# amorim-cleison/sign-language-nlp

Measured on AMD Instinct MI355X. Metric: train seq/s (batch=50,len=48), higher is better.
Workload: dtype bf16x3; 1 GPU; cfg2: Transformer train step E512 H8 N6 F512 batch 50 len 48 |src| 3000 |tgt| 202 dropout 0.1, fwd+CE+bwd+clip(0.5)+SGD(m=.9); launch=eager stream launches (auto: timed both in 9 untimed pre-warmup steps + warmup), per_gpu=independent fit (grid shard)

## Files before the change

### include/slnlp.h

```cpp
#ifndef SLNLP_H
#define SLNLP_H

#include <stdint.h>

#ifdef __cplusplus
extern "C" {
#endif

#define SLNLP_OK 0
#define SLNLP_ERR_INVALID_ARG 1
#define SLNLP_ERR_LAUNCH 2
#define SLNLP_ERR_UNSUPPORTED 3

#define SLNLP_ABI_VERSION 1

const char* slnlp_last_error(void);
int slnlp_abi_version(void);

typedef struct slnlp_gemm_args {
    const float* A; int64_t lda; int32_t a_kmajor;
    const float* B; int64_t ldb; int32_t b_kmajor;
    float* C; int64_t ldc;
    int32_t M, N, K;
    const float* bias;
// ... 5 lines not shown
    int32_t precision;
    int32_t gate_mode;
    const uint16_t* A_hi; const uint16_t* A_lo; int64_t lda_p;
    const uint16_t* B_hi; const uint16_t* B_lo; int64_t ldb_p;
    uint16_t* C_hi; uint16_t* C_lo; int64_t ldc_p;
    int32_t drop_head_dim;
    const float* col_scale;
    uint8_t* C_q8;
    int32_t batch;
    int64_t batch_stride_a, batch_stride_b, batch_stride_c;
} slnlp_gemm_args;

int slnlp_gemm(const slnlp_gemm_args* args, void* stream);
int64_t slnlp_gemm_group_scratch_bytes(const slnlp_gemm_args* jobs, const int32_t* split_k, int njobs);
int slnlp_set_plane_tile(int tile);
int slnlp_set_gemm_ks(int ks);
int slnlp_set_rnn_step_tile(int rows16);
int slnlp_set_fp8_tile(int tile);
int slnlp_gemm_group(const slnlp_gemm_args* jobs, const int32_t* split_k, int njobs, void* scratch,
                     int64_t scratch_bytes, void* stream);
int slnlp_gemm_wd(const slnlp_gemm_args* wgrad, const slnlp_gemm_args* dgrad, void* scratch, int64_t scratch_bytes, void* stream);
int slnlp_gemm_wd_plan(const slnlp_gemm_args* wgrad, const slnlp_gemm_args* dgrad, int32_t* split, int32_t* separate, int32_t* geo_wgrad,
                       int32_t* geo_dgrad);
int slnlp_gemm_rows(const slnlp_gemm_args* args, void* stream);
int slnlp_gemm_rows_ln(const slnlp_gemm_args* args, const float* x, int64_t ldx, const float* gamma, const float* beta, float eps,
                       float* y, float* stats, uint16_t* y_hi, uint16_t* y_lo, int64_t ldp, void* stream);
int slnlp_gemm_rows_bwd(const slnlp_gemm_args* dgrad, const slnlp_gemm_args* wgrad, void* stream);
int slnlp_set_rows_tile(int tile);
int slnlp_quant_rows_fp8(const float* x, int64_t ld, int R, int K, uint8_t* q, int64_t ldq, float* scale, void* stream);
int slnlp_split_planes(const float* x, int64_t ld, int R, int C, uint16_t* hi, uint16_t* lo, int64_t ldp, void* stream);
// ... 518 lines not shown
```

### sign-language-nlp_amd/csrc/gemm_planes.hip

```cpp
#include <algorithm>
#include <vector>

#include "common.hpp"
#include "gemm_jobs.hpp"

namespace slnlp {

typedef __attribute__((ext_vector_type(8))) __bf16 bf16x8;
typedef __attribute__((ext_vector_type(4))) short s16x4;
typedef __attribute__((ext_vector_type(8))) short s16x8;
typedef __attribute__((ext_vector_type(4))) float f32x4;
typedef __attribute__((address_space(3))) void* lds_vp;
typedef __attribute__((address_space(1))) const void* glb_vp;
typedef __attribute__((ext_vector_type(4))) unsigned int u32x4;

constexpr int PT = 64;
constexpr int PTHREADS = 512;

__device__ __forceinline__ int mswz(int k) { return (((k >> 1) & 1) | (((k >> 3) & 1) << 1)) << 1; }

template <bool KMAJOR>
__device__ __forceinline__ int img_off(int row, int k) {
    if (KMAJOR) return row * PT + ((((k >> 3) ^ (row & 7)) << 3) | (k & 7));
    return k * PT + ((((row >> 3) ^ mswz(k)) << 3) | (row & 7));
// ... 71 lines not shown
#define TS_CLK(slot) do { } while (0)
#else
#define TS_CLK(slot) do { if (slot == 1) ts[6] = __builtin_amdgcn_s_memtime(); if (slot == 2) ts[7] = __builtin_amdgcn_s_memtime(); } while (0)
#endif
#define TS_MARK(slot) do { if (threadIdx.x == 0) { ts[slot] = __builtin_amdgcn_s_memrealtime(); \
        TS_CLK(slot); } } while (0)
#else
#define TS_MARK(slot) do { } while (0)
#endif
#if SLNLP_PROBE_FENCES == 128 && defined(SLNLP_PROBE_EPI)
#define TS_EPI(slot) do { if (threadIdx.x == 0) ts[slot] = __builtin_amdgcn_s_memrealtime(); } while (0)
#else
#define TS_EPI(slot) do { } while (0)
#endif

template <int NSPLIT, bool AK, bool BK, int BM, int BN, int BKS, int NST>
__device__ __forceinline__ void plane_kloop(const slnlp_gemm_args& g, unsigned short* smem, int bm0, int bn0, int kt0, int kt1,
                                            bool do_rowsum, f32x4 (&acc)[BM / 64][BN / 32], float (&rowsum)[BM / PT],
                                            unsigned long long* ts) {
    constexpr int NPA = NSPLIT == 3 ? 2 : 1, NPB = NSPLIT >= 2 ? 2 : 1;
    constexpr int SUBM = BM / PT, SUBN = BN / PT;
    constexpr int MT = BM / 64, NT = BN / 32;
    constexpr int IMG_E = PT * BKS;
    constexpr int A_IMGS = NPA * SUBM, B_IMGS = NPB * SUBN;
    constexpr int STAGE = (A_IMGS + B_IMGS) * IMG_E;
    constexpr int PIECES = (A_IMGS + B_IMGS) * BKS / 64;
    static_assert(BKS == 64 || (BM % 128 == 0 && BN % 128 == 0), "32-k stages move 128-row slabs");
    const int tid = threadIdx.x, lane = tid & 63, wave = __builtin_amdgcn_readfirstlane(tid >> 6);
    const int wm0 = (wave >> 1) * (BM / 4), wn0 = (wave & 1) * (BN / 2);
    const int am_last = ((g.M + PT - 1) / PT - 1) * PT, bn_last = ((g.N + PT - 1) / PT - 1) * PT;

    constexpr int APC = BKS == 64 ? SUBM : SUBM / 2, BPC = BKS == 64 ? SUBN : SUBN / 2;
    unsigned aoff[APC], boff[BPC];
#pragma unroll
    for (int q = 0; q < APC; ++q) {
        if constexpr (BKS == 64) aoff[q] = plane_lane_off<AK>(g.lda_p, BM > PT ? min(bm0 + q * PT, am_last) : bm0, wave, lane);
        else aoff[q] = slab32_lane_off<AK>(g.lda_p, bm0 + 2 * q * PT, am_last, wave, lane);
    }
#pragma unroll
    for (int q = 0; q < BPC; ++q) {
        if constexpr (BKS == 64) boff[q] = plane_lane_off<BK>(g.ldb_p, BN > PT ? min(bn0 + q * PT, bn_last) : bn0, wave, lane);
        else boff[q] = slab32_lane_off<BK>(g.ldb_p, bn0 + 2 * q * PT, bn_last, wave, lane);
    }
    constexpr int PSTEP = BKS == 64 ? 1 : 2;
    auto issue = [&](int kt, int stage) {
        const int k0 = (kt < kt1 ? kt : kt0) * BKS;
        const long ka = AK ? (long)k0 : (long)k0 * g.lda_p, kb = BK ? (long)k0 : (long)k0 * g.ldb_p;
        unsigned short* s = smem + stage * STAGE + wave * 512;
#pragma unroll
        for (int q = 0; q < APC; ++q) {
            dma_piece(g.A_hi, ka, aoff[q], s + q * PSTEP * IMG_E);
            if (NPA == 2) dma_piece(g.A_lo, ka, aoff[q], s + (SUBM + q * PSTEP) * IMG_E);
        }
#pragma unroll
        for (int q = 0; q < BPC; ++q) {
            dma_piece(g.B_hi, kb, boff[q], s + (A_IMGS + q * PSTEP) * IMG_E);
            if (NPB == 2) dma_piece(g.B_lo, kb, boff[q], s + (A_IMGS + SUBN + q * PSTEP) * IMG_E);
        }
    };

    for (int t = 0; t < NST - 1; ++t) issue(kt0 + t, t);
    for (int kt = kt0; kt < kt1; ++kt) {
        const int it = kt - kt0;
        asm volatile("s_waitcnt vmcnt(%0)\n\ts_waitcnt lgkmcnt(0)" ::"n"((NST - 2) * PIECES) : "memory");
        __builtin_amdgcn_s_barrier();
        asm volatile("" ::: "memory");
#if SLNLP_PROBE_FENCES == 128
        if (kt == kt0) TS_MARK(1);
#endif
        issue(kt + NST - 1, (it + NST - 1) % NST);
        const unsigned short* s = smem + (it % NST) * STAGE;
#pragma unroll
        for (int kk = 0; kk < BKS / 32; ++kk) {
            constexpr int JB = NT > 4 ? 4 : NT;
            bf16x8 ah[MT], al[MT];
#pragma unroll
            for (int i = 0; i < MT; ++i) {
                const int row = wm0 + 16 * i;
                if constexpr (BKS == 64) {
                    ah[i] = pfrag<AK>(s + (row / PT) * IMG_E, row % PT, kk, lane);
                    if (NPA == 2) al[i] = pfrag<AK>(s + (SUBM + row / PT) * IMG_E, row % PT, kk, lane);
                } else {
                    ah[i] = pfrag32<AK>(s + (row / PT) * IMG_E, row % PT, lane);
                    if (NPA == 2) al[i] = pfrag32<AK>(s + (SUBM + row / PT) * IMG_E, row % PT, lane);
                }
            }
#pragma unroll
            for (int j0 = 0; j0 < NT; j0 += JB) {
                bf16x8 bh[JB], bl[JB];
#pragma unroll
                for (int j = 0; j < JB; ++j) {
                    const int row = wn0 + 16 * (j0 + j);
                    if constexpr (BKS == 64) {
                        bh[j] = pfrag<BK>(s + (A_IMGS + row / PT) * IMG_E, row % PT, kk, lane);
                        if (NPB == 2) bl[j] = pfrag<BK>(s + (A_IMGS + SUBN + row / PT) * IMG_E, row % PT, kk, lane);
                    } else {
                        bh[j] = pfrag32<BK>(s + (A_IMGS + row / PT) * IMG_E, row % PT, lane);
                        if (NPB == 2) bl[j] = pfrag32<BK>(s + (A_IMGS + SUBN + row / PT) * IMG_E, row % PT, lane);
                    }
                }
#pragma unroll
                for (int i = 0; i < MT; ++i)
#pragma unroll
                    for (int j = 0; j < JB; ++j) {
                        f32x4& c = acc[i][j0 + j];
                        if (NPA == 2) c = __builtin_amdgcn_mfma_f32_16x16x32_bf16(al[i], bh[j], c, 0, 0, 0);
                        if (NPB == 2) c = __builtin_amdgcn_mfma_f32_16x16x32_bf16(ah[i], bl[j], c, 0, 0, 0);
                        c = __builtin_amdgcn_mfma_f32_16x16x32_bf16(ah[i], bh[j], c, 0, 0, 0);
                    }
            }
        }
        if (do_rowsum) {
            constexpr int OCT = BKS / 8;
            const int row = tid & 63, kq = ((tid >> 6) % OCT) * 8, sub0 = (tid >> 6) / OCT;
#pragma unroll
            for (int sm = 0; sm < SUBM; sm += 8 / OCT) {
                const int im = sm + sub0;
                float t = 0.f;
#pragma unroll
                for (int k = 0; k < 8; ++k) {
                    const int off = BKS == 64 ? img_off<AK>(row, kq + k) : img32_off<AK>(row, kq + k);
                    t += pbf2f(s[im * IMG_E + off]);
                    if (NPA == 2) t += pbf2f(s[(SUBM + im) * IMG_E + off]);
                }
                if (BKS == 64) rowsum[sm] += t;
                else if (kt & 1) rowsum[sm + 1] += t;
                else rowsum[sm] += t;
            }
        }
    }
}

template <int NSPLIT, int BM, int BN, int BKS, int NST>
__device__ __forceinline__ void plane_tile(const PlaneJob& job, int lid, bool placed, unsigned short* smem) {
    unsigned long long* tsp = nullptr;
#if SLNLP_PROBE_FENCES == 128
    unsigned long long ts[TS_W] = {0, 0, 0, 0, 0, 0, 0, 0};
    struct TsFlush {
        unsigned long long* t;
        __device__ ~TsFlush() {
            if (threadIdx.x == 0) {
                t[4] = __builtin_amdgcn_s_memrealtime();
                unsigned hw;
                asm volatile("s_getreg_b32 %0, hwreg(HW_REG_XCC_ID)" : "=s"(hw));
                t[5] = ((unsigned long long)hw << 32) | blockIdx.x;
                const unsigned i = atomicAdd(&g_ts_n, 1u) & (unsigned)(TS_MAX - 1);
                for (int k = 0; k < TS_W; ++k) g_ts[i][k] = t[k];
            }
        }
    } ts_flush{ts};
    tsp = ts;
    TS_MARK(0);
#endif
    constexpr int SUBM = BM / PT;
    constexpr int MT = BM / 64, NT = BN / 32;
    constexpr int KSUB = PT / BKS;
    const slnlp_gemm_args& g = job.a;
    const int tid = threadIdx.x, lane = tid & 63, wave = __builtin_amdgcn_readfirstlane(tid >> 6);
    const int wm0 = (wave >> 1) * (BM / 4), wn0 = (wave & 1) * (BN / 2);
    const int nks = job.nks;
    int bx, by, ks, tile;
    {
        const int nwg = job.tiles_x * job.tiles_y * nks;
        const int xcd = lid & 7, q = nwg >> 3, r = nwg & 7;
        const int t = placed ? lid : (xcd < r ? xcd * (q + 1) : r * (q + 1) + (xcd - r) * q) + (lid >> 3);
        const int ntiles = job.tiles_x * job.tiles_y;
        ks = t / ntiles;
        tile = t - ks * ntiles;
        constexpr int GR = BM >= 256 ? 2 : BM >= 128 ? 4 : 8;
        const int grp = tile / (GR * job.tiles_x), rem = tile - grp * (GR * job.tiles_x);
        const int rows_here = min(GR, job.tiles_y - grp * GR);
        bx = rem / rows_here;
        by = grp * GR + (rem - bx * rows_here);
        tile = by * job.tiles_x + bx;
// ... 1 lines not shown
    const int bm0 = by * BM, bn0 = bx * BN;
    const int M = g.M, N = g.N, K = g.K;
    const int ktiles = (K + PT - 1) / PT;
    const int kt0 = (int)((long)ktiles * ks / nks) * KSUB, kt1 = (int)((long)ktiles * (ks + 1) / nks) * KSUB;

    f32x4 acc[MT][NT];
#pragma unroll
    for (int i = 0; i < MT; ++i)
#pragma unroll
        for (int j = 0; j < NT; ++j) acc[i][j] = f32x4{0.f, 0.f, 0.f, 0.f};
    const bool do_rowsum = (g.rowsum_a != nullptr) && (bx == 0);
    float rowsum[SUBM];
#pragma unroll
    for (int i = 0; i < SUBM; ++i) rowsum[i] = 0.f;

    if (job.variant == 0) plane_kloop<NSPLIT, true, true, BM, BN, BKS, NST>(g, smem, bm0, bn0, kt0, kt1, do_rowsum, acc, rowsum, tsp);
    else if (job.variant == 1) plane_kloop<NSPLIT, true, false, BM, BN, BKS, NST>(g, smem, bm0, bn0, kt0, kt1, do_rowsum, acc, rowsum, tsp);
    else if (job.variant == 2) plane_kloop<NSPLIT, false, false, BM, BN, BKS, NST>(g, smem, bm0, bn0, kt0, kt1, do_rowsum, acc, rowsum, tsp);
    else if constexpr (NSPLIT == 3) {
        if (job.variant == 3) plane_kloop<2, true, false, BM, BN, BKS, NST + 1>(g, smem, bm0, bn0, kt0, kt1, do_rowsum, acc, rowsum, tsp);
        else plane_kloop<2, false, false, BM, BN, BKS, NST + 1>(g, smem, bm0, bn0, kt0, kt1, do_rowsum, acc, rowsum, tsp);
    }
    TS_MARK(2);
    asm volatile("s_waitcnt vmcnt(0)" ::: "memory");
    __builtin_amdgcn_s_barrier();
    float* rs = reinterpret_cast<float*>(smem);
    int* flag = reinterpret_cast<int*>(smem) + SUBM * PTHREADS;
    float rs_row = 0.f;
    if (do_rowsum) {
        if (BKS == 64) {
#pragma unroll
            for (int sm = 0; sm < SUBM; ++sm) rs[(sm * 8 + (tid >> 6)) * PT + (tid & 63)] = rowsum[sm];
        } else {
#pragma unroll
            for (int sm = 0; sm < SUBM; sm += 2) {
                const int im = sm + (tid >> 8), o = (tid >> 6) & 3;
// ... 74 lines not shown
    if (g.drop_p > 0.f) dkey = dropout_key(g.rng, g.drop_site);
#pragma unroll 1
    for (int ch = 0; ch < ECH; ++ch) {
        __syncthreads();
        if (ECH == 1 || wm0 / ER == ch) {
            const int lr0 = wm0 - ch * ER + crow, lc0 = wn0 + ccol;
#pragma unroll
            for (int i = 0; i < MT; ++i)
#pragma unroll
                for (int j = 0; j < NT; ++j)
#pragma unroll
                    for (int r = 0; r < 4; ++r) stg[(lr0 + 16 * i + r) * SLD + lc0 + 16 * j] = acc[i][j][r];
#if defined(SLNLP_PROBE_EPI) && SLNLP_PROBE_EPI == 2
            if (ch == 0) TS_EPI(6);
#endif
            if (early) {
                static_assert(NT % 2 == 0, "column tiles in pairs");
#pragma unroll 1
                for (int t = 0; t < MT * (NT / 2); ++t) {
                    const int lm0 = lr0 + 16 * (t / (NT / 2)), ln0 = lc0 + 32 * (t % (NT / 2));
                    const int gm0 = bm0 + ch * ER + lm0, gn0 = bn0 + ln0;
                    if (gn0 >= N || gm0 >= M) continue;
                    float v[2][4], gt[2][4];
#pragma unroll
                    for (int h = 0; h < 2; ++h)
#pragma unroll
                        for (int r = 0; r < 4; ++r) {
                            v[h][r] = stg[(lm0 + r) * SLD + ln0 + 16 * h];
                            gt[h][r] = 1.f;
                            if (g.gate && gm0 + r < M && gn0 + 16 * h < N) gt[h][r] = g.gate[(long)(gm0 + r) * g.ldg + gn0 + 16 * h];
                        }
// ... 269 lines not shown
                if (g.C) g.C[(long)gm * g.ldc + gn] = v;
                if (g.C_hi) {
                    unsigned short h, l;
                    split_bf16(v, h, l);
                    g.C_hi[(long)gm * g.ldc_p + gn] = h;
                    if (g.C_lo) g.C_lo[(long)gm * g.ldc_p + gn] = l;
                }
                if (g.C_q8) g.C_q8[(long)gm * g.ldc_p + gn] = (unsigned char)(pack_fp8x4(v, 0.f, 0.f, 0.f) & 0xFFu);
            }
        }
}

constexpr int PLACE_JOB_BITS = 12, PLACE_JOBS = 1 << PLACE_JOB_BITS;

struct GeoInfo { int bm, bn, bks, nst; };
constexpr int NGEO = 4;
constexpr GeoInfo GEO[NGEO] = {{64, 64, 64, 2}, {128, 128, 64, 2}, {128, 128, 32, 2}, {256, 256, 32, 2}};

template <int NSPLIT, int G>
__global__ __launch_bounds__(PTHREADS) void gemm_planes_kernel(const PlaneGroupParams P, const PlaneJob* __restrict__ tab,
                                                               const int* __restrict__ blockmap) {
    extern __shared__ __attribute__((aligned(16))) unsigned short smem[];
    PlaneJob job;
    int lid;
    bool placed = false;
    if (tab) {
        const int m = blockmap[blockIdx.x];
        if (m < 0) return;
        job = tab[m & (PLACE_JOBS - 1)];
        lid = m >> PLACE_JOB_BITS;
        placed = true;
    } else {
// ... 15 lines not shown
constexpr size_t plane_lds(int geo) {
    const size_t ring3 = (size_t)GEO[geo].nst * 2 * (GEO[geo].bm + GEO[geo].bn) * GEO[geo].bks * sizeof(unsigned short);
    const size_t ring2 = (size_t)(GEO[geo].nst + 1) * (GEO[geo].bm + 2 * GEO[geo].bn) * GEO[geo].bks * sizeof(unsigned short);
    const size_t ring = ring3 > ring2 ? ring3 : ring2;
    const size_t image = ((size_t)(GEO[geo].bm > 128 ? 128 : GEO[geo].bm) * (GEO[geo].bn + 4) + GEO[geo].bn) * sizeof(float);
    return ring > image ? ring : image;
}
constexpr int GROUP_COUNTERS = 4096;

struct Q8GeoInfo { int bm, bn, nst; };
constexpr int NQGEO = 2;
constexpr Q8GeoInfo QGEO[NQGEO] = {{64, 64, 4}, {128, 128, 2}};

template <int G>
__global__ __launch_bounds__(PTHREADS) void plane_splitk_reduce_kernel(const PlaneJob job_in) {
    constexpr int BM = GEO[G].bm, BN = GEO[G].bn, MT = BM / 64, NT = BN / 32, TILE_FLOATS = BM * BN, SC = 17;
    PlaneJob job = job_in;
    launder(job.a);
    const slnlp_gemm_args& g = job.a;
    const int tid = threadIdx.x, lane = tid & 63, wave = tid >> 6;
    const int tile = blockIdx.x / (MT * NT), slab = blockIdx.x - tile * (MT * NT), i = slab / NT, j = slab - i * NT;
    const int by = tile / job.tiles_x, bx = tile - by * job.tiles_x, nks = job.nks;
    const int wm0 = (wave >> 1) * (BM / 4), wn0 = (wave & 1) * (BN / 2);
    u32x4 p[WD_MAX_SPLITK];
#pragma unroll
    for (int s = 0; s < WD_MAX_SPLITK; ++s) {
        if (s < nks) {
            const __amdgpu_buffer_rsrc_t q =
                __builtin_amdgcn_make_buffer_rsrc(job.part + ((long)tile * nks + s) * TILE_FLOATS, 0, TILE_FLOATS * 4, 0x00020000);
            p[s] = __builtin_amdgcn_raw_buffer_load_b128(q, tid * 16, slab * PTHREADS * 16, SC);
// ... 56 lines not shown
static int q8_geo_of_knob(int knob) { return knob == 64 ? 0 : knob == 128 ? 1 : -1; }
static std::atomic<int> g_q8_geo{[] { const char* e = getenv("SLNLP_Q8_TILE"); return q8_geo_of_knob(e ? atoi(e) : 0); }()};
static int q8_geo_auto(const PlaneJob* jobs, int njobs) {
    const int forced = g_q8_geo.load(std::memory_order_relaxed);
    if (forced >= 0) return forced;
    long units = 0;
    for (int i = 0; i < njobs; ++i) units += (long)ceil_div(jobs[i].a.M, 128) * ceil_div(jobs[i].a.N, 128);
    return units >= 512 ? 1 : 0;
}

static int splitk_mode() {
    static const int mode = [] { const char* e = getenv("SLNLP_SPLITK_MODE"); return e ? atoi(e) : 0; }();
    return mode;
}

static int geo_of_knob(int knob) { return knob == 64 ? 0 : knob == 128 ? 1 : knob == 12832 ? 2 : knob == 256 ? 3 : -1; }
static std::atomic<int> g_plane_geo{[] { const char* e = getenv("SLNLP_PLANE_TILE"); return geo_of_knob(e ? atoi(e) : 0); }()};
constexpr int BIG_TILE_MIN_UNITS = 200;

constexpr int TWO_PER_CU_UNITS = 300;
struct LaunchShape {
    long units128 = 0, units256 = 0;
    int min_k = 1 << 30;
    bool forward = true;
    int njobs = 0;
};
static void shape_add(LaunchShape& s, const slnlp_gemm_args& a, int nks) {
    if (nks < 1) nks = 1;
    s.units128 += (long)ceil_div(a.M, 128) * ceil_div(a.N, 128) * nks;
    s.units256 += (long)ceil_div(a.M, 256) * ceil_div(a.N, 256) * nks;
    s.min_k = std::min(s.min_k, a.K / nks);
    s.forward = s.forward && a.a_kmajor && a.b_kmajor && nks == 1 && a.precision != 2;
    ++s.njobs;
}
static int plane_geo_auto(const LaunchShape& s) {
    const int forced = g_plane_geo.load(std::memory_order_relaxed);
    if (forced >= 0) return forced;
    if (s.units128 < BIG_TILE_MIN_UNITS) return 0;
    if (s.forward && s.min_k >= 1024 && (s.units256 >= 512 || s.min_k >= 2048) && s.units256 * 100 >= (s.units256 + 255) / 256 * 256 * 85) return 3;
    if (s.njobs == 1 && !s.forward && s.min_k >= 2048 && s.units256 >= 192 && s.units256 * 100 >= (s.units256 + 255) / 256 * 256 * 85) return 3;
    return (s.min_k >= 1024 || s.units128 >= TWO_PER_CU_UNITS) ? 2 : 1;
}
int plane_geo_for(const slnlp_gemm_args* jobs, const int* split_k, int njobs) {
    LaunchShape s;
    for (int i = 0; i < njobs; ++i) {
        if (jobs[i].precision == 8) return 0;
        shape_add(s, jobs[i], split_k ? split_k[i] : 1);
    }
    return plane_geo_auto(s);
}

int gemm_planes_init() {
    static DeviceOnce once;
    return once.run([]() -> int {
        bool ok = true;
        for (int prec = 1; prec <= 3; prec += 2)
            for (int geo = 0; geo < NGEO; ++geo)
                ok = ok && hipFuncSetAttribute(gemm_planes_kernel_ptr(prec, geo), hipFuncAttributeMaxDynamicSharedMemorySize, (int)plane_lds(geo)) == hipSuccess;
        for (int geo = 0; geo < NQGEO; ++geo)
            ok = ok && hipFuncSetAttribute(q8_kernel_ptr(geo), hipFuncAttributeMaxDynamicSharedMemorySize, (int)q8_lds(geo)) == hipSuccess;
        if (!ok) {
            set_error("gemm_planes_init: cannot raise dynamic LDS limit: %s", hipGetErrorString(hipGetLastError()));
            return SLNLP_ERR_LAUNCH;
        }
        return 0;
    });
}

static int check_plane_job(const slnlp_gemm_args& a) {
    SLNLP_CHECK_ARG(a.A_hi && a.B_hi, "gemm_planes: operand planes required");
    SLNLP_CHECK_ARG(a.C || a.C_hi, "gemm_planes: no output");
    SLNLP_CHECK_ARG(a.M > 0 && a.N > 0 && a.K > 0, "gemm_planes: bad shape M=%d N=%d K=%d", a.M, a.N, a.K);
    if (a.precision == 8) {
        SLNLP_CHECK_ARG(a.a_kmajor && a.b_kmajor, "gemm_planes: precision 8 (fp8) is built for k-major operands (forward products)");
        SLNLP_CHECK_ARG(a.lda_p % 128 == 0 && a.ldb_p % 128 == 0 && a.lda_p >= a.K && a.ldb_p >= a.K,
                        "gemm_planes: fp8 plane row strides must be multiples of 128 bytes and cover K");
        SLNLP_CHECK_ARG(!a.gate && !a.rowsum_a && a.drop_head_dim == 0, "gemm_planes: fp8 jobs take bias / relu / dropout / residual only");
        SLNLP_CHECK_ARG((((uintptr_t)a.A_hi | (uintptr_t)a.B_hi) & 15) == 0, "gemm_planes: planes must be 16-byte aligned");
// ... 318 lines not shown
    if (hipLaunchKernel(b.fn, dim3(blocks), dim3(PTHREADS), args, b.lds, s) != hipSuccess) {
        set_error("gemm_planes (batch): %s", hipGetErrorString(hipGetLastError()));
        return SLNLP_ERR_LAUNCH;
    }
    if (timed >= 0) launch_timer_end(timed, s, blocks, (int)b.jobs.size(), b.geo);
    return 0;
}
int plane_geo_forced() { return g_plane_geo.load(std::memory_order_relaxed); }

template <int NSPLIT>
static const void* kernel_of(int geo) {
    switch (geo) {
        case 1: return (const void*)gemm_planes_kernel<NSPLIT, 1>;
        case 2: return (const void*)gemm_planes_kernel<NSPLIT, 2>;
        case 3: return (const void*)gemm_planes_kernel<NSPLIT, 3>;
        default: return (const void*)gemm_planes_kernel<NSPLIT, 0>;
    }
}
const void* gemm_planes_kernel_ptr(int precision, int geo) { return precision == 1 ? kernel_of<1>(geo) : kernel_of<3>(geo); }

int gemm_planes(const slnlp_gemm_args& a, hipStream_t s) { return gemm_planes_group(&a, nullptr, 1, nullptr, 0, s); }

__device__ __forceinline__ void split_planes_body(const float* __restrict__ x, long ld, int R, int C, unsigned short* __restrict__ hi,
                                                  unsigned short* __restrict__ lo, long ldp) {
    const long n4 = (long)R * (C >> 2);
    for (long i = blockIdx.x * 256L + threadIdx.x; i < n4; i += (long)gridDim.x * 256) {
        const int r = (int)(i / (C >> 2)), c = (int)(i % (C >> 2)) << 2;
        const float4 v = *reinterpret_cast<const float4*>(x + (long)r * ld + c);
        const float f[4] = {v.x, v.y, v.z, v.w};
        unsigned short h[4], l[4];
// ... 45 lines not shown
                   hipStream_t st) {
    SLNLP_CHECK_ARG(x && q && scale && R > 0, "quant_rows_fp8: bad arguments");
    SLNLP_CHECK_ARG(row_table || (K > 0 && K % 4 == 0 && ld % 4 == 0 && ldq % 4 == 0 && ldq >= K), "quant_rows_fp8: K, ld, ldq must be multiples of 4");
    return zlaunch(quant_rows_fp8_kernel, dim3(ceil_div(R, 4)), 256, 0, st, "quant_rows_fp8", x, (long)ld, R, K, q, (long)ldq, scale,
                   (const QuantRow*)row_table);
}

}

extern "C" int slnlp_quant_rows_fp8(const float* x, int64_t ld, int R, int K, uint8_t* q, int64_t ldq, float* scale, void* stream) {
    return slnlp::quant_rows_fp8(x, ld, R, K, q, ldq, scale, nullptr, (hipStream_t)stream);
}

extern "C" int slnlp_set_plane_tile(int tile) {
    if (tile != 0 && slnlp::geo_of_knob(tile) < 0) {
        slnlp::set_error("set_plane_tile: %d (0 = automatic, 64, 128, 12832 = 128 x 128 with 32-k stages, 256 = 256 x 256 with 32-k stages)", tile);
        return SLNLP_ERR_INVALID_ARG;
    }
    slnlp::g_plane_geo.store(slnlp::geo_of_knob(tile), std::memory_order_relaxed);
    return 0;
}

extern "C" int slnlp_set_fp8_tile(int tile) {
    if (tile != 0 && slnlp::q8_geo_of_knob(tile) < 0) {
        slnlp::set_error("set_fp8_tile: %d (0 = automatic, 64 or 128)", tile);
        return SLNLP_ERR_INVALID_ARG;
    }
    slnlp::g_q8_geo.store(slnlp::q8_geo_of_knob(tile), std::memory_order_relaxed);
    return 0;
}

extern "C" int64_t slnlp_gemm_group_scratch_bytes(const slnlp_gemm_args* jobs, const int32_t* split_k, int njobs) {
    if (!jobs || njobs < 1) return 0;
    return (int64_t)slnlp::gemm_group_scratch_bytes(jobs, split_k, njobs);
}
// ... 50 lines not shown
```

### sign-language-nlp_amd/slnlp/_lib.py

```python
import ctypes as C
import os

_HERE = os.path.dirname(os.path.abspath(__file__))
LIB_PATH = os.path.join(os.path.dirname(_HERE), "lib",
                        f"libslnlp_probe{os.environ['SLNLP_PROBE_LIB']}.so" if os.environ.get("SLNLP_PROBE_LIB") else "libslnlp.so")

i32, i64, f32, vp = C.c_int32, C.c_int64, C.c_float, C.c_void_p


class GemmArgs(C.Structure):
    _fields_ = [("A", vp), ("lda", i64), ("a_kmajor", i32),
                ("B", vp), ("ldb", i64), ("b_kmajor", i32),
                ("C", vp), ("ldc", i64),
                ("M", i32), ("N", i32), ("K", i32),
                ("bias", vp), ("relu", i32),
                ("gate", vp), ("ldg", i64), ("gate_scale", f32),
                ("drop_p", f32), ("drop_site", i32), ("rng", vp),
                ("resid", vp), ("ldr", i64),
                ("rowsum_a", vp), ("precision", i32), ("gate_mode", i32),
                ("A_hi", vp), ("A_lo", vp), ("lda_p", i64), ("B_hi", vp), ("B_lo", vp), ("ldb_p", i64),
                ("C_hi", vp), ("C_lo", vp), ("ldc_p", i64), ("drop_head_dim", i32),
                ("col_scale", vp), ("C_q8", vp),
                ("batch", i32), ("batch_stride_a", i64), ("batch_stride_b", i64), ("batch_stride_c", i64)]

# ... 196 lines not shown
    "slnlp_tf_debug_layout": (i32, [vp, C.c_char_p, i64]),
    "slnlp_tf_set_destroy_sync": (i32, [vp, i32]),
    "slnlp_tf_set_criterion": (i32, [vp, vp, f32, i32, vp]),
    "slnlp_tf_set_update": (i32, [vp, i32, f32, f32, i32]),
    "slnlp_tf_set_param_groups": (i32, [vp, i32, vp, vp, i32, vp, vp, vp]),
    "slnlp_tf_set_averaging": (i32, [vp, vp, vp, i32, f32]),
    "slnlp_tf_set_dmem_batched": (i32, [vp, i32]),
    "slnlp_tf_set_dec_ln_fused": (i32, [vp, i32]),
    "slnlp_set_stream_policy": (i32, [i32]),
    "slnlp_set_thread_stream_policy": (i32, [i32]),
    "slnlp_set_backward_passes": (i32, [i32, i32]),
    "slnlp_get_backward_passes": (i32, [C.POINTER(i32), C.POINTER(i32)]),
    "slnlp_launch_timer_start": (i32, [i32]),
    "slnlp_launch_timer_stop": (i32, [C.POINTER(TimedLaunch), i32]),
    "slnlp_set_plane_tile": (i32, [i32]),
    "slnlp_set_gemm_ks": (i32, [i32]),
    "slnlp_set_fp8_tile": (i32, [i32]),
    "slnlp_tf_lockstep_workspace_bytes": (i64, [vp, i32]),
    "slnlp_tf_lockstep_create": (i32, [vp, i32, vp, i64, vp, vp]),
    "slnlp_tf_lockstep_destroy": (None, [vp]),
    "slnlp_tf_lockstep_set_data": (i32, [vp, i32, vp, vp, i64, vp, vp, vp]),
    "slnlp_tf_lockstep_step": (i32, [vp, i32, i64, i32, i32, i32, C.c_float, C.c_float, vp]),
    "slnlp_tf_lockstep_epoch": (i32, [vp, i32, i32, i32, C.c_float, C.c_float, vp]),
    "slnlp_tf_lockstep_num_launches": (i32, [vp, i32, i32, i32]),
    "slnlp_tf_lockstep_set_adam": (i32, [vp, vp, f32, f32, f32, f32]),
    "slnlp_tf_lockstep_set_lr_table": (i32, [vp, vp, i32, vp]),
    "slnlp_tf_lockstep_set_order": (i32, [vp, i32, vp, i64, vp]),
    "slnlp_tf_lockstep_set_averaging": (i32, [vp, vp, vp, i32, f32]),
    "slnlp_tf_lockstep_set_destroy_sync": (i32, [vp, i32]),
    "slnlp_rnn_lockstep_workspace_bytes": (i64, [vp, i32]),
# ... 101 lines not shown
```

### sign-language-nlp_amd/slnlp/ops.py

```python
import ctypes as C
import math
import numbers

import torch

from . import _lib, _packed
from ._lib import GemmArgs, check, load, ptr, stream_ptr


def make_rng(seed=0, step=0, device="cuda"):
    return torch.tensor([seed, step], dtype=torch.int64, device=device)


def gemm(A, B, *, M, N, K, a_kmajor=True, b_kmajor=True, lda=None, ldb=None, out=None, ldc=None,
         bias=None, relu=False, gate=None, gate_scale=1.0, gate_mode=0, drop_p=0.0, drop_site=0, rng=None,
         resid=None, rowsum_a=None, precision=3):
    _lib.require_gpu()
    lda = lda if lda is not None else (K if a_kmajor else M)
    ldb = ldb if ldb is not None else (K if b_kmajor else N)
    ldc = ldc if ldc is not None else N
    if out is None:
        out = torch.empty(M, ldc, dtype=torch.float32, device=A.device)
    a = GemmArgs()
    a.A, a.lda, a.a_kmajor = ptr(A), lda, int(a_kmajor)
# ... 64 lines not shown
    a.bias, a.relu, a.rowsum_a = ptr(bias), int(relu), ptr(rowsum_a)
    a.resid, a.ldr = ptr(resid), (resid.stride(0) if resid is not None else 0)
    return a, out


def gemm_group(jobs, split_k=None, scratch=None):
    _lib.require_gpu()
    n = len(jobs)
    arr = (GemmArgs * n)(*jobs)
    sk = (C.c_int32 * n)(*(split_k or [1] * n))
    if scratch is None:
        nbytes = int(load().slnlp_gemm_group_scratch_bytes(arr, sk, n))
        scratch = torch.zeros(nbytes, dtype=torch.uint8, device="cuda")
    check(load().slnlp_gemm_group(arr, sk, n, ptr(scratch), scratch.numel(), stream_ptr()), "gemm_group")
    return scratch


def gemm_wd_plan(jw, jd):
    v = [C.c_int32(0) for _ in range(4)]
    check(load().slnlp_gemm_wd_plan(C.byref(jw), C.byref(jd), *[C.byref(x) for x in v]), "gemm_wd_plan")
    return tuple(int(x.value) for x in v)


def gemm_wd(jw, jd, scratch=None):
    _lib.require_gpu()
    if scratch is None:
        arr = (GemmArgs * 2)(jw, jd)
        sk = (C.c_int32 * 2)(8, 1)
        scratch = torch.zeros(int(load().slnlp_gemm_group_scratch_bytes(arr, sk, 2)), dtype=torch.uint8, device="cuda")
    check(load().slnlp_gemm_wd(C.byref(jw), C.byref(jd), ptr(scratch), scratch.numel(), stream_ptr()), "gemm_wd")
# ... 1614 lines not shown
```

Baseline: 21370 seq/s.

## Add 96x64 plane GEMM tile for solo launches with k-major A

Adds a fifth plane-GEMM geometry, 96x64 with a 3-stage pipeline and a 2x4 wave grid. It is picked automatically for single-job launches whose 64x64 tile count falls between one and two waves over 256 CUs but whose 96x64 tile count fits in one wave, so the second partial wave of tiles goes away. This takes a half-panel A load split across waves, per-wave vmcnt waits, an NT==1 epilogue path and an occupancy check at init. In exchange, fewer MFMA tiles per wave and the odd-sized panel may lower per-tile efficiency.

```diff
diff --git a/include/slnlp.h b/include/slnlp.h
--- a/include/slnlp.h
+++ b/include/slnlp.h
@@ -43,6 +43,7 @@
 int slnlp_gemm(const slnlp_gemm_args* args, void* stream);
 int64_t slnlp_gemm_group_scratch_bytes(const slnlp_gemm_args* jobs, const int32_t* split_k, int njobs);
 int slnlp_set_plane_tile(int tile);
+int slnlp_plane_geo(const slnlp_gemm_args* jobs, const int32_t* split_k, int njobs);
 int slnlp_set_gemm_ks(int ks);
 int slnlp_set_rnn_step_tile(int rows16);
 int slnlp_set_fp8_tile(int tile);
diff --git a/sign-language-nlp_amd/csrc/gemm_planes.hip b/sign-language-nlp_amd/csrc/gemm_planes.hip
--- a/sign-language-nlp_amd/csrc/gemm_planes.hip
+++ b/sign-language-nlp_amd/csrc/gemm_planes.hip
@@ -109,29 +109,52 @@
 #define TS_EPI(slot) do { } while (0)
 #endif
 
+template <int BM, int BN>
+struct WaveGrid {
+    static constexpr int WN = BM % 64 == 0 ? 2 : 4, WM = 8 / WN, WN_SH = WN == 2 ? 1 : 2;
+    static constexpr int MT = BM / WM / 16, NT = BN / WN / 16;
+    static constexpr int SUBM = (BM + PT - 1) / PT;
+    static_assert(BM % (16 * WM) == 0 && BN % (16 * WN) == 0, "whole MFMA tiles per wave");
+    static __device__ __forceinline__ int wm0(int wave) { return (wave >> WN_SH) * (BM / WM); }
+    static __device__ __forceinline__ int wn0(int wave) { return (wave & (WN - 1)) * (BN / WN); }
+};
+
+__device__ __forceinline__ unsigned plane_lane_off_clamped(long ld, int row0, int row_max, int wave, int lane) {
+    const int line = 8 * wave + (lane >> 3), ps = lane & 7;
+    return (unsigned)(((long)min(row0 + line, row_max) * ld + ((ps ^ (line & 7)) << 3)) * 2);
+}
+
 template <int NSPLIT, bool AK, bool BK, int BM, int BN, int BKS, int NST>
 __device__ __forceinline__ void plane_kloop(const slnlp_gemm_args& g, unsigned short* smem, int bm0, int bn0, int kt0, int kt1,
-                                            bool do_rowsum, f32x4 (&acc)[BM / 64][BN / 32], float (&rowsum)[BM / PT],
-                                            unsigned long long* ts) {
+                                            bool do_rowsum, f32x4 (&acc)[WaveGrid<BM, BN>::MT][WaveGrid<BM, BN>::NT],
+                                            float (&rowsum)[WaveGrid<BM, BN>::SUBM], unsigned long long* ts) {
     constexpr int NPA = NSPLIT == 3 ? 2 : 1, NPB = NSPLIT >= 2 ? 2 : 1;
-    constexpr int SUBM = BM / PT, SUBN = BN / PT;
-    constexpr int MT = BM / 64, NT = BN / 32;
+    using WG = WaveGrid<BM, BN>;
+    constexpr int SUBM = WG::SUBM, SUBN = BN / PT;
+    constexpr int MT = WG::MT, NT = WG::NT;
     constexpr int IMG_E = PT * BKS;
-    constexpr int A_IMGS = NPA * SUBM, B_IMGS = NPB * SUBN;
-    constexpr int STAGE = (A_IMGS + B_IMGS) * IMG_E;
-    constexpr int PIECES = (A_IMGS + B_IMGS) * BKS / 64;
+    constexpr int A_E = BM * BKS, B_E = BN * BKS;
+    constexpr int A_LO = A_E, B_HI = NPA * A_E, B_LO = B_HI + B_E;
+    constexpr int STAGE = NPA * A_E + NPB * B_E;
+    constexpr bool HALF_A = BM % PT != 0;
+    constexpr int PIECES = HALF_A ? NPA + 1 + NPB * SUBN : (NPA * SUBM + NPB * SUBN) * BKS / 64;
+    constexpr int PIECES_HI = HALF_A && NPA == 1 ? PIECES - 1 : PIECES;
     static_assert(BKS == 64 || (BM % 128 == 0 && BN % 128 == 0), "32-k stages move 128-row slabs");
+    static_assert(!HALF_A || (AK && BKS == 64 && BM == PT + PT / 2), "the 96-row panel is built for k-major A and 64-k stages");
     const int tid = threadIdx.x, lane = tid & 63, wave = __builtin_amdgcn_readfirstlane(tid >> 6);
-    const int wm0 = (wave >> 1) * (BM / 4), wn0 = (wave & 1) * (BN / 2);
+    const int wm0 = WG::wm0(wave), wn0 = WG::wn0(wave);
     const int am_last = ((g.M + PT - 1) / PT - 1) * PT, bn_last = ((g.N + PT - 1) / PT - 1) * PT;
 
-    constexpr int APC = BKS == 64 ? SUBM : SUBM / 2, BPC = BKS == 64 ? SUBN : SUBN / 2;
+    constexpr int APC = HALF_A ? 1 : BKS == 64 ? SUBM : SUBM / 2, BPC = BKS == 64 ? SUBN : SUBN / 2;
     unsigned aoff[APC], boff[BPC];
+    unsigned aoff_half = 0;
 #pragma unroll
     for (int q = 0; q < APC; ++q) {
-        if constexpr (BKS == 64) aoff[q] = plane_lane_off<AK>(g.lda_p, BM > PT ? min(bm0 + q * PT, am_last) : bm0, wave, lane);
+        if constexpr (HALF_A) aoff[q] = plane_lane_off_clamped(g.lda_p, bm0, am_last + PT - 1, wave, lane);
+        else if constexpr (BKS == 64) aoff[q] = plane_lane_off<AK>(g.lda_p, BM > PT ? min(bm0 + q * PT, am_last) : bm0, wave, lane);
         else aoff[q] = slab32_lane_off<AK>(g.lda_p, bm0 + 2 * q * PT, am_last, wave, lane);
     }
+    if constexpr (HALF_A) aoff_half = plane_lane_off_clamped(g.lda_p, bm0 + PT, am_last + PT - 1, wave & 3, lane);
 #pragma unroll
     for (int q = 0; q < BPC; ++q) {
         if constexpr (BKS == 64) boff[q] = plane_lane_off<BK>(g.ldb_p, BN > PT ? min(bn0 + q * PT, bn_last) : bn0, wave, lane);
@@ -145,19 +168,25 @@
 #pragma unroll
         for (int q = 0; q < APC; ++q) {
             dma_piece(g.A_hi, ka, aoff[q], s + q * PSTEP * IMG_E);
-            if (NPA == 2) dma_piece(g.A_lo, ka, aoff[q], s + (SUBM + q * PSTEP) * IMG_E);
+            if (NPA == 2) dma_piece(g.A_lo, ka, aoff[q], s + (A_LO + q * PSTEP * IMG_E));
+        }
+        if constexpr (HALF_A) {
+            unsigned short* sh = smem + stage * STAGE + IMG_E + (wave & 3) * 512;
+            if (wave < 4) dma_piece(g.A_hi, ka, aoff_half, sh);
+            else if (NPA == 2) dma_piece(g.A_lo, ka, aoff_half, sh + A_LO);
         }
 #pragma unroll
         for (int q = 0; q < BPC; ++q) {
-            dma_piece(g.B_hi, kb, boff[q], s + (A_IMGS + q * PSTEP) * IMG_E);
-            if (NPB == 2) dma_piece(g.B_lo, kb, boff[q], s + (A_IMGS + SUBN + q * PSTEP) * IMG_E);
+            dma_piece(g.B_hi, kb, boff[q], s + (B_HI + q * PSTEP * IMG_E));
+            if (NPB == 2) dma_piece(g.B_lo, kb, boff[q], s + (B_LO + q * PSTEP * IMG_E));
         }
     };
 
     for (int t = 0; t < NST - 1; ++t) issue(kt0 + t, t);
     for (int kt = kt0; kt < kt1; ++kt) {
         const int it = kt - kt0;
-        asm volatile("s_waitcnt vmcnt(%0)\n\ts_waitcnt lgkmcnt(0)" ::"n"((NST - 2) * PIECES) : "memory");
+        if (PIECES_HI == PIECES || wave < 4) asm volatile("s_waitcnt vmcnt(%0)\n\ts_waitcnt lgkmcnt(0)" ::"n"((NST - 2) * PIECES) : "memory");
+        else asm volatile("s_waitcnt vmcnt(%0)\n\ts_waitcnt lgkmcnt(0)" ::"n"((NST - 2) * PIECES_HI) : "memory");
         __builtin_amdgcn_s_barrier();
         asm volatile("" ::: "memory");
 #if SLNLP_PROBE_FENCES == 128
@@ -174,10 +203,10 @@
                 const int row = wm0 + 16 * i;
                 if constexpr (BKS == 64) {
                     ah[i] = pfrag<AK>(s + (row / PT) * IMG_E, row % PT, kk, lane);
-                    if (NPA == 2) al[i] = pfrag<AK>(s + (SUBM + row / PT) * IMG_E, row % PT, kk, lane);
+                    if (NPA == 2) al[i] = pfrag<AK>(s + (A_LO + (row / PT) * IMG_E), row % PT, kk, lane);
                 } else {
                     ah[i] = pfrag32<AK>(s + (row / PT) * IMG_E, row % PT, lane);
-                    if (NPA == 2) al[i] = pfrag32<AK>(s + (SUBM + row / PT) * IMG_E, row % PT, lane);
+                    if (NPA == 2) al[i] = pfrag32<AK>(s + (A_LO + (row / PT) * IMG_E), row % PT, lane);
                 }
             }
 #pragma unroll
@@ -187,11 +216,11 @@
                 for (int j = 0; j < JB; ++j) {
                     const int row = wn0 + 16 * (j0 + j);
                     if constexpr (BKS == 64) {
-                        bh[j] = pfrag<BK>(s + (A_IMGS + row / PT) * IMG_E, row % PT, kk, lane);
-                        if (NPB == 2) bl[j] = pfrag<BK>(s + (A_IMGS + SUBN + row / PT) * IMG_E, row % PT, kk, lane);
+                        bh[j] = pfrag<BK>(s + (B_HI + (row / PT) * IMG_E), row % PT, kk, lane);
+                        if (NPB == 2) bl[j] = pfrag<BK>(s + (B_LO + (row / PT) * IMG_E), row % PT, kk, lane);
                     } else {
-                        bh[j] = pfrag32<BK>(s + (A_IMGS + row / PT) * IMG_E, row % PT, lane);
-                        if (NPB == 2) bl[j] = pfrag32<BK>(s + (A_IMGS + SUBN + row / PT) * IMG_E, row % PT, lane);
+                        bh[j] = pfrag32<BK>(s + (B_HI + (row / PT) * IMG_E), row % PT, lane);
+                        if (NPB == 2) bl[j] = pfrag32<BK>(s + (B_LO + (row / PT) * IMG_E), row % PT, lane);
                     }
                 }
 #pragma unroll
@@ -211,12 +240,15 @@
 #pragma unroll
             for (int sm = 0; sm < SUBM; sm += 8 / OCT) {
                 const int im = sm + sub0;
+                if constexpr (HALF_A) {
+                    if (im * PT + row >= BM) continue;
+                }
                 float t = 0.f;
 #pragma unroll
                 for (int k = 0; k < 8; ++k) {
                     const int off = BKS == 64 ? img_off<AK>(row, kq + k) : img32_off<AK>(row, kq + k);
                     t += pbf2f(s[im * IMG_E + off]);
-                    if (NPA == 2) t += pbf2f(s[(SUBM + im) * IMG_E + off]);
+                    if (NPA == 2) t += pbf2f(s[A_LO + im * IMG_E + off]);
                 }
                 if (BKS == 64) rowsum[sm] += t;
                 else if (kt & 1) rowsum[sm + 1] += t;
@@ -247,12 +279,13 @@
     tsp = ts;
     TS_MARK(0);
 #endif
-    constexpr int SUBM = BM / PT;
-    constexpr int MT = BM / 64, NT = BN / 32;
+    using WG = WaveGrid<BM, BN>;
+    constexpr int SUBM = WG::SUBM;
+    constexpr int MT = WG::MT, NT = WG::NT;
     constexpr int KSUB = PT / BKS;
     const slnlp_gemm_args& g = job.a;
     const int tid = threadIdx.x, lane = tid & 63, wave = __builtin_amdgcn_readfirstlane(tid >> 6);
-    const int wm0 = (wave >> 1) * (BM / 4), wn0 = (wave & 1) * (BN / 2);
+    const int wm0 = WG::wm0(wave), wn0 = WG::wn0(wave);
     const int nks = job.nks;
     int bx, by, ks, tile;
     {
@@ -284,12 +317,20 @@
 #pragma unroll
     for (int i = 0; i < SUBM; ++i) rowsum[i] = 0.f;
 
-    if (job.variant == 0) plane_kloop<NSPLIT, true, true, BM, BN, BKS, NST>(g, smem, bm0, bn0, kt0, kt1, do_rowsum, acc, rowsum, tsp);
-    else if (job.variant == 1) plane_kloop<NSPLIT, true, false, BM, BN, BKS, NST>(g, smem, bm0, bn0, kt0, kt1, do_rowsum, acc, rowsum, tsp);
-    else if (job.variant == 2) plane_kloop<NSPLIT, false, false, BM, BN, BKS, NST>(g, smem, bm0, bn0, kt0, kt1, do_rowsum, acc, rowsum, tsp);
-    else if constexpr (NSPLIT == 3) {
-        if (job.variant == 3) plane_kloop<2, true, false, BM, BN, BKS, NST + 1>(g, smem, bm0, bn0, kt0, kt1, do_rowsum, acc, rowsum, tsp);
-        else plane_kloop<2, false, false, BM, BN, BKS, NST + 1>(g, smem, bm0, bn0, kt0, kt1, do_rowsum, acc, rowsum, tsp);
+    if constexpr (BM % PT != 0) {
+        if (job.variant == 0) plane_kloop<NSPLIT, true, true, BM, BN, BKS, NST>(g, smem, bm0, bn0, kt0, kt1, do_rowsum, acc, rowsum, tsp);
+        else if (job.variant == 1) plane_kloop<NSPLIT, true, false, BM, BN, BKS, NST>(g, smem, bm0, bn0, kt0, kt1, do_rowsum, acc, rowsum, tsp);
+        else if constexpr (NSPLIT == 3) {
+            if (job.variant == 3) plane_kloop<2, true, false, BM, BN, BKS, NST + 1>(g, smem, bm0, bn0, kt0, kt1, do_rowsum, acc, rowsum, tsp);
+        }
+    } else {
+        if (job.variant == 0) plane_kloop<NSPLIT, true, true, BM, BN, BKS, NST>(g, smem, bm0, bn0, kt0, kt1, do_rowsum, acc, rowsum, tsp);
+        else if (job.variant == 1) plane_kloop<NSPLIT, true, false, BM, BN, BKS, NST>(g, smem, bm0, bn0, kt0, kt1, do_rowsum, acc, rowsum, tsp);
+        else if (job.variant == 2) plane_kloop<NSPLIT, false, false, BM, BN, BKS, NST>(g, smem, bm0, bn0, kt0, kt1, do_rowsum, acc, rowsum, tsp);
+        else if constexpr (NSPLIT == 3) {
+            if (job.variant == 3) plane_kloop<2, true, false, BM, BN, BKS, NST + 1>(g, smem, bm0, bn0, kt0, kt1, do_rowsum, acc, rowsum, tsp);
+            else plane_kloop<2, false, false, BM, BN, BKS, NST + 1>(g, smem, bm0, bn0, kt0, kt1, do_rowsum, acc, rowsum, tsp);
+        }
     }
     TS_MARK(2);
     asm volatile("s_waitcnt vmcnt(0)" ::: "memory");
@@ -394,7 +435,38 @@
 #if defined(SLNLP_PROBE_EPI) && SLNLP_PROBE_EPI == 2
             if (ch == 0) TS_EPI(6);
 #endif
-            if (early) {
+            if constexpr (NT % 2 != 0) {
+                static_assert(NT == 1, "one column tile per wave");
+                if (early) {
+#pragma unroll 1
+                    for (int t = 0; t < MT; ++t) {
+                        const int lm0 = lr0 + 16 * t, gm0 = bm0 + ch * ER + lm0, gn0 = bn0 + lc0;
+                        if (gn0 >= N || gm0 >= M) continue;
+                        float v[4], gt[4];
+#pragma unroll
+                        for (int r = 0; r < 4; ++r) {
+                            v[r] = stg[(lm0 + r) * SLD + lc0];
+                            gt[r] = 1.f;
+                            if (g.gate && gm0 + r < M) gt[r] = g.gate[(long)(gm0 + r) * g.ldg + gn0];
+                        }
+                        const float bias = sbias[lc0];
+                        uint4 bits = make_uint4(0, 0, 0, 0);
+                        if (g.drop_p > 0.f) bits = dropout_bits8(dkey, (unsigned)gm0 >> 2, drop_cc((unsigned)gn0));
+                        const int h = drop_half((unsigned)gn0);
+#pragma unroll
+                        for (int r = 0; r < 4; ++r) {
+                            float x = v[r] + bias;
+                            if (g.relu == 1) x = fmaxf(x, 0.f);
+                            else if (g.relu == 2) x = tanhf(x);
+                            if (g.gate) x = g.gate_mode == 1 ? x * (1.f - gt[r] * gt[r]) : (gt[r] > 0.f ? x * g.gate_scale : 0.f);
+                            if (g.drop_p > 0.f) x = (pick_lot(bits, h, r) >= job.drop_thr) ? x * job.drop_scale : 0.f;
+                            v[r] = x;
+                        }
+#pragma unroll
+                        for (int r = 0; r < 4; ++r) stg[(lm0 + r) * SLD + lc0] = v[r];
+                    }
+                }
+            } else if (early) {
                 static_assert(NT % 2 == 0, "column tiles in pairs");
 #pragma unroll 1
                 for (int t = 0; t < MT * (NT / 2); ++t) {
@@ -694,8 +766,8 @@
 constexpr int PLACE_JOB_BITS = 12, PLACE_JOBS = 1 << PLACE_JOB_BITS;
 
 struct GeoInfo { int bm, bn, bks, nst; };
-constexpr int NGEO = 4;
-constexpr GeoInfo GEO[NGEO] = {{64, 64, 64, 2}, {128, 128, 64, 2}, {128, 128, 32, 2}, {256, 256, 32, 2}};
+constexpr int NGEO = 5, GEO_SOLO96 = 4;
+constexpr GeoInfo GEO[NGEO] = {{64, 64, 64, 2}, {128, 128, 64, 2}, {128, 128, 32, 2}, {256, 256, 32, 2}, {96, 64, 64, 3}};
 
 template <int NSPLIT, int G>
 __global__ __launch_bounds__(PTHREADS) void gemm_planes_kernel(const PlaneGroupParams P, const PlaneJob* __restrict__ tab,
@@ -741,6 +813,7 @@
 
 template <int G>
 __global__ __launch_bounds__(PTHREADS) void plane_splitk_reduce_kernel(const PlaneJob job_in) {
+    static_assert(GEO[G].bm % 64 == 0, "split-K geometries only (4 x 2 wave grid)");
     constexpr int BM = GEO[G].bm, BN = GEO[G].bn, MT = BM / 64, NT = BN / 32, TILE_FLOATS = BM * BN, SC = 17;
     PlaneJob job = job_in;
     launder(job.a);
@@ -827,28 +900,37 @@
     return mode;
 }
 
-static int geo_of_knob(int knob) { return knob == 64 ? 0 : knob == 128 ? 1 : knob == 12832 ? 2 : knob == 256 ? 3 : -1; }
+static int geo_of_knob(int knob) { return knob == 64 ? 0 : knob == 128 ? 1 : knob == 12832 ? 2 : knob == 256 ? 3 : knob == 96 ? GEO_SOLO96 : -1; }
 static std::atomic<int> g_plane_geo{[] { const char* e = getenv("SLNLP_PLANE_TILE"); return geo_of_knob(e ? atoi(e) : 0); }()};
 constexpr int BIG_TILE_MIN_UNITS = 200;
 
 constexpr int TWO_PER_CU_UNITS = 300;
 struct LaunchShape {
     long units128 = 0, units256 = 0;
+    long units64 = 0, units96 = 0;
     int min_k = 1 << 30;
     bool forward = true;
+    bool a_rows = true;
+    bool solo = false;
     int njobs = 0;
 };
 static void shape_add(LaunchShape& s, const slnlp_gemm_args& a, int nks) {
     if (nks < 1) nks = 1;
     s.units128 += (long)ceil_div(a.M, 128) * ceil_div(a.N, 128) * nks;
     s.units256 += (long)ceil_div(a.M, 256) * ceil_div(a.N, 256) * nks;
+    s.units64 += (long)ceil_div(a.M, 64) * ceil_div(a.N, 64) * nks;
+    s.units96 += (long)ceil_div(a.M, 96) * ceil_div(a.N, 64) * nks;
     s.min_k = std::min(s.min_k, a.K / nks);
     s.forward = s.forward && a.a_kmajor && a.b_kmajor && nks == 1 && a.precision != 2;
+    s.a_rows = s.a_rows && a.a_kmajor && nks == 1;
     ++s.njobs;
 }
+constexpr int CUS = 256;
 static int plane_geo_auto(const LaunchShape& s) {
     const int forced = g_plane_geo.load(std::memory_order_relaxed);
-    if (forced >= 0) return forced;
+    const bool can96 = s.solo && s.njobs == 1 && s.a_rows;
+    if (forced >= 0) return forced == GEO_SOLO96 && !can96 ? 0 : forced;
+    if (can96 && s.units64 > CUS && s.units64 <= 2 * CUS && s.units96 <= CUS) return GEO_SOLO96;
     if (s.units128 < BIG_TILE_MIN_UNITS) return 0;
     if (s.forward && s.min_k >= 1024 && (s.units256 >= 512 || s.min_k >= 2048) && s.units256 * 100 >= (s.units256 + 255) / 256 * 256 * 85) return 3;
     if (s.njobs == 1 && !s.forward && s.min_k >= 2048 && s.units256 >= 192 && s.units256 * 100 >= (s.units256 + 255) / 256 * 256 * 85) return 3;
@@ -860,6 +942,7 @@
         if (jobs[i].precision == 8) return 0;
         shape_add(s, jobs[i], split_k ? split_k[i] : 1);
     }
+    s.solo = njobs == 1;
     return plane_geo_auto(s);
 }
 
@@ -875,6 +958,17 @@
         if (!ok) {
             set_error("gemm_planes_init: cannot raise dynamic LDS limit: %s", hipGetErrorString(hipGetLastError()));
             return SLNLP_ERR_LAUNCH;
+        }
+        for (int prec = 1; prec <= 3; prec += 2) {
+            int per_cu = 0;
+            if (hipOccupancyMaxActiveBlocksPerMultiprocessor(&per_cu, gemm_planes_kernel_ptr(prec, GEO_SOLO96), PTHREADS, plane_lds(GEO_SOLO96)) != hipSuccess) {
+                (void)hipGetLastError();
+                continue;
+            }
+            if (per_cu > 1) {
+                set_error("gemm_planes_init: the 96 x 64 tile must run one workgroup per CU, the runtime reports %d", per_cu);
+                return SLNLP_ERR_LAUNCH;
+            }
         }
         return 0;
     });
@@ -1223,6 +1317,7 @@
         case 1: return (const void*)gemm_planes_kernel<NSPLIT, 1>;
         case 2: return (const void*)gemm_planes_kernel<NSPLIT, 2>;
         case 3: return (const void*)gemm_planes_kernel<NSPLIT, 3>;
+        case 4: return (const void*)gemm_planes_kernel<NSPLIT, 4>;
         default: return (const void*)gemm_planes_kernel<NSPLIT, 0>;
     }
 }
@@ -1298,11 +1393,17 @@
 
 extern "C" int slnlp_set_plane_tile(int tile) {
     if (tile != 0 && slnlp::geo_of_knob(tile) < 0) {
-        slnlp::set_error("set_plane_tile: %d (0 = automatic, 64, 128, 12832 = 128 x 128 with 32-k stages, 256 = 256 x 256 with 32-k stages)", tile);
+        slnlp::set_error("set_plane_tile: %d (0 = automatic, 64, 128, 12832 = 128 x 128 with 32-k stages, 256 = 256 x 256 with 32-k stages, "
+                         "96 = 96 x 64 for solo launches with k-major A)", tile);
         return SLNLP_ERR_INVALID_ARG;
     }
     slnlp::g_plane_geo.store(slnlp::geo_of_knob(tile), std::memory_order_relaxed);
     return 0;
+}
+
+extern "C" int slnlp_plane_geo(const slnlp_gemm_args* jobs, const int32_t* split_k, int njobs) {
+    if (!jobs || njobs < 1) return 0;
+    return slnlp::plane_geo_for(jobs, split_k, njobs);
 }
 
 extern "C" int slnlp_set_fp8_tile(int tile) {
diff --git a/sign-language-nlp_amd/slnlp/_lib.py b/sign-language-nlp_amd/slnlp/_lib.py
--- a/sign-language-nlp_amd/slnlp/_lib.py
+++ b/sign-language-nlp_amd/slnlp/_lib.py
@@ -234,6 +234,7 @@
     "slnlp_launch_timer_start": (i32, [i32]),
     "slnlp_launch_timer_stop": (i32, [C.POINTER(TimedLaunch), i32]),
     "slnlp_set_plane_tile": (i32, [i32]),
+    "slnlp_plane_geo": (i32, [vp, vp, i32]),
     "slnlp_set_gemm_ks": (i32, [i32]),
     "slnlp_set_fp8_tile": (i32, [i32]),
     "slnlp_tf_lockstep_workspace_bytes": (i64, [vp, i32]),
diff --git a/sign-language-nlp_amd/slnlp/ops.py b/sign-language-nlp_amd/slnlp/ops.py
--- a/sign-language-nlp_amd/slnlp/ops.py
+++ b/sign-language-nlp_amd/slnlp/ops.py
@@ -102,6 +102,13 @@
         scratch = torch.zeros(nbytes, dtype=torch.uint8, device="cuda")
     check(load().slnlp_gemm_group(arr, sk, n, ptr(scratch), scratch.numel(), stream_ptr()), "gemm_group")
     return scratch
+
+
+def plane_geo(jobs, split_k=None):
+    n = len(jobs)
+    arr = (GemmArgs * n)(*jobs)
+    sk = (C.c_int32 * n)(*(split_k or [1] * n))
+    return int(load().slnlp_plane_geo(arr, sk, n))
 
 
 def gemm_wd_plan(jw, jd):
```

Result: faster. 21590 seq/s, median of 6 (+1.0%).
